# jtdaugherty/flux

Measured on AMD Instinct MI355X. Metric: Msamples/sec on demo2.yml (fixed spp), higher is better.
Workload: dtype f64

## Files before the change

### flux_amd/build.py

```python
import os
import shutil
import subprocess
import sys

ROOT = os.path.dirname(os.path.dirname(os.path.abspath(__file__)))
CSRC = os.path.join(ROOT, "flux_amd", "csrc")
HIP_SOURCES = ["abi.hip", "multi.hip", "tables.hip", "render.hip", "bvh.cpp", "scene_build.cpp", "launch_plan.cpp"]
HIP_HEADERS = ["flux_ctx.h", "scene_build.h", "joining_thread.h", "flux_device.h", "flux_plan.h", "flux_rng.h", "flux_tables.h", "flux_bvh.h", "flux_math.h",
               "flux_math_coeffs.h", "render_body.inc"]
HIP_LIB = os.path.join(ROOT, "flux_amd", "libflux_hip.so")

HIP_FLAGS = ["--offload-arch=gfx950", "-O3", "-std=c++17", "-fPIC", "-shared", "-ffp-contract=off",
             "-fno-fast-math", "-Wall", "-Wno-unused-function",
             "-mllvm", "-disable-machine-licm"]


def _newer(target, deps):
    if not os.path.exists(target):
        return True
    t = os.path.getmtime(target)
    return any(os.path.getmtime(d) > t for d in deps)


def _hipcc():
    for cand in (os.environ.get("HIPCC"), shutil.which("hipcc"), "/opt/rocm/bin/hipcc"):
        if cand and os.path.exists(cand):
            return cand
    raise RuntimeError("hipcc not found (set HIPCC)")


KERNEL_FILES = ["render.hip", "render_body.inc", "tables.hip", "flux_device.h", "flux_plan.h", "flux_bvh.h", "flux_math.h",
                "flux_math_coeffs.h", "flux_rng.h", "flux_tables.h"]


def build_id(extra_flags=()):
    import hashlib

    def digest(names):
        h = hashlib.sha256()
        h.update(" ".join(HIP_FLAGS + list(extra_flags)).encode())
        for n in names:
            path = os.path.join(ROOT, "include", n) if n == "flux_abi.h" else os.path.join(CSRC, n)
            h.update(n.encode() + b"\0")
            with open(path, "rb") as f:
                h.update(f.read())
        return h.hexdigest()[:16]
    return f"lib:{digest(sorted(set(HIP_SOURCES + HIP_HEADERS + ['flux_abi.h'])))} kernels:{digest(KERNEL_FILES)}"


def _id_flag(extra_flags=()):
    return "-DFLUX_BUILD_ID=\"" + build_id(extra_flags) + "\""


def build_variant(out_path, extra_flags, verbose=False):
    srcs = [os.path.join(CSRC, s) for s in HIP_SOURCES]
    flags = [f for f in HIP_FLAGS if not (f == "-ffp-contract=off" and any(x.startswith("-ffp-contract") for x in extra_flags))]
    cmd = [_hipcc()] + flags + list(extra_flags) + [_id_flag(extra_flags), "-o", out_path] + srcs
    if verbose:
        print(" ".join(cmd), file=sys.stderr)
    subprocess.run(cmd, check=True, cwd=CSRC)
    return out_path


def build_hip(force=False, verbose=False):
    srcs = [os.path.join(CSRC, s) for s in HIP_SOURCES]
    deps = srcs + [os.path.join(CSRC, h) for h in HIP_HEADERS] + [os.path.join(ROOT, "include", "flux_abi.h")]
    if not force and not _newer(HIP_LIB, deps):
        return HIP_LIB
    cmd = [_hipcc()] + HIP_FLAGS + [_id_flag(), "-o", HIP_LIB] + srcs
    if verbose:
        print(" ".join(cmd), file=sys.stderr)
    subprocess.run(cmd, check=True, cwd=CSRC)
    return HIP_LIB


HOST_DIR = os.path.join(ROOT, "flux_amd", "host")
HOST_SOURCES = ["flux_host.cpp", "yaml_lite.cpp", "cbor.cpp", "flux_net.cpp"]
HOST_BINARIES = {"flux": "flux_cli.cpp", "flux_host_test": "flux_host_test.cpp", "sampler_debug": "sampler_debug.cpp",
                 "flux_node": "flux_node.cpp"}


def build_host(force=False, verbose=False):
    build_hip(force=False, verbose=verbose)
    outs = []
    common = [os.path.join(HOST_DIR, s) for s in HOST_SOURCES]
# ... 18 lines not shown
```

### flux_amd/csrc/flux_device.h

```cpp
#pragma once
#include <hip/hip_runtime.h>
#include <stdint.h>

#include "flux_bvh.h"


#ifndef FLUX_UNI_SPHERES
#define FLUX_UNI_SPHERES 2
#endif
#ifndef FLUX_BVH_WIDE_MAX_STACK
#define FLUX_BVH_WIDE_MAX_STACK 48
#endif
#ifndef FLUX_MAX_WAVES_PER_PIXEL
#define FLUX_MAX_WAVES_PER_PIXEL 4
#endif
#ifndef FLUX_MIN_SAMPLES_PER_WAVE
#define FLUX_MIN_SAMPLES_PER_WAVE 4096
#endif

namespace flux {

constexpr int kHemiDoubles = 4;
constexpr double kTMin = 0.0005;
constexpr double kPi = 3.14159265358979323846264338327950288;
constexpr double kInvPi = 1.0 / kPi;

constexpr int kShapeSphere = 0;
constexpr int kShapePlane = 1;
constexpr int kShapeDisk = 2;
constexpr int kShapeBox = 3;
constexpr int kMatMatte = 0;
constexpr int kMatEmissive = 1;
constexpr int kMatReflective = 2;
constexpr int kMatGlossy = 3;
constexpr int kMatDielectric = 4;

struct DevShape {
    double px, py, pz;
    double rr;
    double c0x, c0y, c0z;
    double radius;
    double c1x, c1y, c1z;
    double inv;
    int32_t kind;
    int32_t pad0;
    double inv_rad;
    double pad1[2];
};
static_assert(sizeof(DevShape) == 128, "DevShape layout");

struct DevMaterial {
    double fr, fg, fb;
    double exponent;
    double inv_e1;
    int32_t kind;
    int32_t exp_parity;
    double pad1[2];
// ... 77 lines not shown
    const double *hemi;
    const double *gloss;
    const int32_t *rowperm;
    const int32_t *invperm;
    double *out;
    int32_t first_row, row_stride, num_rows;
    int32_t n_mats;
    unsigned long long *stats;
    const DevTri *tris;
    const DevNode *nodes;
    const DevNodeQ *nodesq;
    float bvh_qmin[3], bvh_qstep[3];
    const DevNode4Q *nodes4;
    const DevLeafRec *leaves;
    int32_t bvh4_stack;
    int32_t mat_bits;
    int32_t n_tris;
    int32_t bvh_stack;
    const DevScanSphere *fsph;
    const DevScanPlane *fpln;
    const DevHitRec *frec;
    const DevScanSphere32 *fsph32;
    const DevShape *sshapes;
    int32_t n_sph, n_pln;
    double bvh_mag;
    int32_t set_first, set_stride, set_count, out_by_set;
    int32_t slot_first, slot_stride;
    int32_t glossy_long;
    int32_t self_skip;
    int32_t n_uni, uni_idx[2];
    int32_t unit_dirs;
    int32_t env_short, pad_env;
    double env_radius;
    double t_min, env_deep;
    double env_px, env_py, env_pz, env_rr;
    double env_eps;
    const DevScanSphere32 *f32_half, *f32_top;
    int32_t f32_groups;
    uint32_t f32_valid;
    double fwx, fwy, fwz;
    const double *pxc;
    const DevSetRows *set_rows;
    double exp2c[12];
    const DevScanDisk *fdsk;
    int32_t n_dsk;
    int32_t has_diel;
    const double2 *glossx;
    const int32_t *gx_off;
    int32_t gx_stride, n_gloss_exp;
    const DevScanBox *fbox;
    int32_t n_box;
    int32_t tput_bits;
    const double *tput;
};

__host__ __device__ inline int hit_records(const RenderParams &p) { return p.n_sph + p.n_pln + p.n_dsk + 6 * p.n_box; }

}
```

### flux_amd/csrc/render_body.inc

```

#undef FLUX_STAGE
#if FLUX_FAST
#define FLUX_STAGE() __builtin_amdgcn_sched_barrier(0)
#else
#define FLUX_STAGE() ((void)0)
#endif

struct Ray {
    double ox, oy, oz, dx, dy, dz;
};

typedef const __attribute__((address_space(4))) RenderParams *ParamsInKernarg;
static_assert(sizeof(DevMaterial) % 16 == 0, "the bounce-weight records behind the materials are read as double2");
__device__ __forceinline__ const RenderParams &relaunder_params(uint32_t tick) {
    ParamsInKernarg p = (ParamsInKernarg)__builtin_amdgcn_kernarg_segment_ptr();
    asm("" : "+s"(p) : "s"(tick));
    return *(const RenderParams *)p;
}

__device__ __forceinline__ unsigned long long ballot64(bool b) { return __builtin_amdgcn_ballot_w64(b); }
__device__ __forceinline__ bool any64(bool b) { return __builtin_amdgcn_ballot_w64(b) != 0ull; }
__device__ __forceinline__ bool all64(bool b) { return __builtin_amdgcn_ballot_w64(!b) == 0ull; }

typedef double flux_d2 __attribute__((ext_vector_type(2)));
// ... 348 lines not shown
        filter_pair_step(F, S[0], cand);
    }
    const DevScanSphere32 *g = P.f32_top;
    for (int n = P.f32_groups; n > 0; --n) {
        g -= 4;
        DevScanSphere32 S[4];
#pragma unroll
        for (int j = 0; j < 4; ++j) S[j] = g[j];
#pragma unroll
        for (int j = 3; j >= 0; --j) filter_pair_step(F, S[j], cand);
    }
    return cand;
}

#if FLUX_FAST
__device__ __forceinline__ bool box_z_nan_miss(const RenderParams &P, const Ray &r, int k) {
    const DevShape &S = P.shapes[P.frec[k].orig_id];
    return r.oz == S.c0z || r.oz == S.c1z;
}

__device__ __forceinline__ double sphere_hb(double tx, double ty, double tz, double ux, double uy, double uz) {
    return __builtin_fma(tz, uz, __builtin_fma(ty, uy, tx * ux));
}

__device__ __forceinline__ void scan_disks(const RenderParams &P, const Ray &r, double tmin, int &best, int &best_id, double &tb) {
    for (int j = 0; j < P.n_dsk; ++j) {
        const DevScanDisk &S = P.fdsk[j];
        double t;
        if (disk_hit(S, r, tmin, t) && (best < 0 || t < tb || (t == tb && S.id < best_id))) {
            best = P.n_sph + P.n_pln + j;
            best_id = S.id;
            tb = t;
        }
    }
}

__device__ __forceinline__ void scan_boxes(const RenderParams &P, const Ray &r, double tmin, int &best, int &best_id, double &tb) {
    if (P.n_box <= 0) return;
    const BoxRay A = box_ray(r);
    const int rec0 = P.n_sph + P.n_pln + P.n_dsk;
    for (int j = 0; j < P.n_box; ++j) {
        const DevScanBox &S = P.fbox[j];
        double t;
        int face;
        if (box_shape_hit(S.c0x, S.c0y, S.c0z, S.c1x, S.c1y, S.c1z, r, A, tmin, t, face) &&
            (best < 0 || t < tb || (t == tb && S.id < best_id))) {
            best = rec0 + 6 * j + face;
            best_id = S.id;
            tb = t;
        }
    }
}

template <bool ENV_SHORT = false, bool LDS_SCENE = false, bool MAX32 = false, bool TYP = false, int ZF = -1>
__device__ __forceinline__ void scan_shapes_fast(const RenderParams &P, const Ray &r, int self, int &best, double &tb,
                                                 long long *lap = nullptr, const char *fsph_lds = nullptr) {
    (void)fsph_lds;
    int best_id = -1;
    const double tmin = P.t_min;
    int j0 = 0;
    if (P.n_pln > 0) {
        const DevScanPlane &S = P.fpln[0];
        const double num = (S.px - r.ox) * S.nx + (S.py - r.oy) * S.ny + (S.pz - r.oz) * S.nz;
        const double den = r.dx * S.nx + r.dy * S.ny + r.dz * S.nz;
        const double t = num / den;
        const bool take = t > tmin;
        best = take ? P.n_sph : -1;
        best_id = S.id;
        tb = (ENV_SHORT || take) ? t : tb;
        j0 = 1;
    }
    for (int j = j0; j < P.n_pln; ++j) {
        const DevScanPlane &S = P.fpln[j];
        const double num = (S.px - r.ox) * S.nx + (S.py - r.oy) * S.ny + (S.pz - r.oz) * S.nz;
        const double den = r.dx * S.nx + r.dy * S.ny + r.dz * S.nz;
        const double t = num / den;
        if (t > tmin && (best < 0 || t < tb)) {
            best = P.n_sph + j;
            best_id = S.id;
            tb = t;
        }
    }
    if (!TYP) {
        scan_disks(P, r, tmin, best, best_id, tb);
        scan_boxes(P, r, tmin, best, best_id, tb);
    }
    const bool p_unit_dirs = TYP ? true : P.unit_dirs != 0;
    const bool p_env_short = TYP ? true : P.env_short != 0;
    const int p_n_uni = TYP ? 1 : P.n_uni;
    double rs = 1.0, ux = r.dx, uy = r.dy, uz = r.dz;
    if (!p_unit_dirs) {
        const double dd = r.dx * r.dx + r.dy * r.dy + r.dz * r.dz;
        rs = fastmath::frsqrt(dd);
        ux = r.dx * rs;
        uy = r.dy * rs;
        uz = r.dz * rs;
    }
    const bool zflat = r.dz == 0.0;
    const bool any_zflat = ZF == 0 ? false : any64(zflat);
    const bool f32_filter = (TYP && ENV_SHORT) ? true : P.fsph32 != nullptr;
    float oof;
    const FilterRay32 F32 = filter_ray32_f(r.ox, r.oy, r.oz, ux, uy, uz, oof);
    const bool big = ZF == 0 ? false : !(oof < 1e30f);
    if (ZF != 0 && !(oof < 0.999e6f)) self = -1;
    lap_stamp(lap, 2);
    const int n_groups_end = MAX32 ? ((TYP || P.n_sph > 0) ? 1 : 0) : P.n_sph;
    for (int base = 0; base < n_groups_end; base += 32) {
        const int lim = MAX32 ? P.n_sph : ((P.n_sph - base) < 32 ? (P.n_sph - base) : 32);
        uint32_t cand = 0;
        if (f32_filter) {
            cand = MAX32 ? sphere_filter32_laid_out(P, F32) : sphere_filter32(P, F32, base, lim);
            const uint32_t valid_bits = MAX32 ? P.f32_valid : (lim == 32 ? 0xffffffffu : (1u << lim) - 1u);
            cand = big ? valid_bits : (cand & valid_bits);
            const uint32_t sb = (uint32_t)(self - base);
            cand &= ~(sb < 32u ? 1u << sb : 0u);
        } else
        {
#pragma unroll 4
        for (int k = 0; k < lim; ++k) {
            const DevScanSphere S = P.fsph[base + k];
            const double tx = r.ox - S.px, ty = r.oy - S.py, tz = r.oz - S.pz;
            const double hb = sphere_hb(tx, ty, tz, ux, uy, uz);
            const double c = __builtin_fma(tx, tx, __builtin_fma(ty, ty, __builtin_fma(tz, tz, -S.rr)));
            const double dq = __builtin_fma(hb, hb, -c);
            const int hq = __double2hiint(dq);
            const int hc = __double2hiint(c);
            const int hmin = min(hc, __double2hiint(hb));
            if (hq >= 0 && hmin <= 0) cand |= 1u << k;
        }
        }
        if (any_zflat) {
            if (zflat)
                for (uint32_t m = cand; m;) {
                    const int k = __builtin_ctz(m);
                    m &= m - 1;
                    if (box_z_nan_miss(P, r, base + k)) cand &= ~(1u << k);
                }
        }
        lap_stamp(lap, 3);
        uint32_t todo = cand;
        if (todo) {
            auto record = [&](int k) {
                if constexpr (LDS_SCENE)
                    return *reinterpret_cast<const DevScanSphere *>(fsph_lds + (uint32_t)(base + k) * (uint32_t)sizeof(DevScanSphere));
                else
                    return *reinterpret_cast<const DevScanSphere *>(
                        reinterpret_cast<const char *>(P.fsph) + (uint32_t)(base + k) * (uint32_t)sizeof(DevScanSphere));
            };
            int k = __builtin_ctz(todo);
            todo &= todo - 1;
            DevScanSphere Sk = record(k);
            for (;;) {
                FLUX_TRIP(P, 11);
                FLUX_CENSUS(P, 4);
                const double tx = r.ox - Sk.px, ty = r.oy - Sk.py, tz = r.oz - Sk.pz;
                const double hb = sphere_hb(tx, ty, tz, ux, uy, uz);
                const double c = __builtin_fma(tx, tx, __builtin_fma(ty, ty, __builtin_fma(tz, tz, -Sk.rr)));
                const double dq = __builtin_fma(hb, hb, -c);
                if (dq >= 0.0) {
                    const double e = fastmath::fsqrt_nonneg(dq);
                    double t = (-hb - e) * rs;
                    if (!(t > tmin)) t = (-hb + e) * rs;
                    if (t > tmin) {
                        bool take = best < 0 || t < tb;
                        if (!take && t == tb && best >= P.n_sph) take = P.frec[base + k].orig_id < best_id;
                        if (take) {
                            best = base + k;
                            tb = t;
                        }
                    }
                }
                if (!todo) break;
                k = __builtin_ctz(todo);
                todo &= todo - 1;
                Sk = record(k);
            }
        }
        lap_stamp(lap, 4);
    }
    if (f32_filter) {
        for (int j = 0; j < p_n_uni; ++j) {
            FLUX_CENSUS(P, 5);
            const int k = P.uni_idx[j];
            const DevScanSphere S = TYP ? DevScanSphere{P.env_px, P.env_py, P.env_pz, P.env_rr} : P.fsph[k];
            const double tx = r.ox - S.px, ty = r.oy - S.py, tz = r.oz - S.pz;
            const double hb = sphere_hb(tx, ty, tz, ux, uy, uz);
            const double c = __builtin_fma(tx, tx, __builtin_fma(ty, ty, __builtin_fma(tz, tz, -S.rr)));
            const double dq = __builtin_fma(hb, hb, -c);
            if (ENV_SHORT && p_env_short && p_unit_dirs && !any_zflat) {
                const bool deep = c < P.env_deep;
                const double s = tb + hb;
                const double s2 = s * s;
                const bool close = fabs(dq - s2) <= P.env_eps * (dq + s2);
                if (((ballot64(!deep)) | (ballot64(best >= 0) & ballot64(close))) == 0ull) {
                    if (best < 0 || (s > 0.0 && dq < s2)) {
                        best = k;
                        tb = 2.0 * P.env_radius;
                    }
                    continue;
                }
            }
            const double e = fastmath::fsqrt_nonneg(__builtin_fmax(dq, 0.0));
            double t = (-hb - e) * rs;
            if (!(t > tmin)) t = (-hb + e) * rs;
            bool ok = dq >= 0.0 && t > tmin;
            if (any_zflat) {
                if (zflat && box_z_nan_miss(P, r, k)) ok = false;
            }
            if (ok) {
                bool take = best < 0 || t < tb;
                if (!take && t == tb) take = best >= P.n_sph ? P.frec[k].orig_id < best_id : k < best;
                if (take) {
                    best = k;
                    tb = t;
                }
            }
        }
    }
}
#endif

template <bool STATS, bool TRIS>
__device__ __forceinline__ int scene_hit(const RenderParams &P, const Ray &r, int self, double &t_out, int &slot_out,
                                         int *tstack, int stride, Stats &st) {
    int best = -1;
    int bslot = -1;
    double tb = 0.0;
#if FLUX_FAST
    scan_shapes_fast(P, r, self, best, tb);
    const int best_rec = best;
    if (TRIS) best = best >= 0 ? 0 : -1;
#else
    const double ax = 1.0 / r.dx, ay = 1.0 / r.dy, az = 1.0 / r.dz;
    const double a = r.dx * r.dx + r.dy * r.dy + r.dz * r.dz;
    const double denom = 2.0 * a;
    const auto box_hit_strict = [&](const DevShape &S) {
        double lox = (S.c0x - r.ox) * ax, hix = (S.c1x - r.ox) * ax;
        double loy = (S.c0y - r.oy) * ay, hiy = (S.c1y - r.oy) * ay;
        double loz = (S.c0z - r.oz) * az, hiz = (S.c1z - r.oz) * az;
        double tx_min = ax >= 0.0 ? lox : hix, tx_max = ax >= 0.0 ? hix : lox;
        double ty_min = ay >= 0.0 ? loy : hiy, ty_max = ay >= 0.0 ? hiy : loy;
        double tz_min = az >= 0.0 ? loz : hiz, tz_max = az >= 0.0 ? hiz : loz;
        const double t0 = __builtin_fmax(tx_min, __builtin_fmax(ty_min, tz_min));
        const double t1 = __builtin_fmin(tx_max, __builtin_fmin(ty_max, tz_max));
        return t0 < t1 && t1 > kTMin && !__builtin_isunordered(tz_min, tz_max);
    };
    const auto sphere_hit_strict = [&](const DevShape &S) {
        V3 temp = mk(r.ox - S.px, r.oy - S.py, r.oz - S.pz);
        double b = 2.0 * (temp.x * r.dx + temp.y * r.dy + temp.z * r.dz);
        double c = dot(temp, temp) - S.rr;
        double disc = b * b - 4.0 * a * c;
        if (!(disc < 0.0)) {
            double e = sqrt(disc);
            double t = (-b - e) / denom;
            bool ok = t > kTMin;
            if (!ok) {
                t = (-b + e) / denom;
                ok = t > kTMin;
            }
            if (ok) consider(t, S.pad0, -1, best, bslot, tb);
        }
    };
    if (P.fsph32 != nullptr) {
        for (int j = 0; j < P.n_pln; ++j) {
            const DevScanPlane &S = P.fpln[j];
            double num = (S.px - r.ox) * S.nx + (S.py - r.oy) * S.ny + (S.pz - r.oz) * S.nz;
            double den = r.dx * S.nx + r.dy * S.ny + r.dz * S.nz;
            double t = num / den;
            if (t > kTMin) consider(t, S.id, -1, best, bslot, tb);
        }
        for (int j = 0; j < P.n_dsk; ++j) {
// ... 289 lines not shown
                    if (rdotwi != rdotwi) lobe = rdotwi;
                    const double pdf = lobe * ndotwi;
                    fr *= lobe;
                    fg *= lobe;
                    fb *= lobe;
                    scale = ndotwi / pdf;
                }
            }
        }
    }
    if (p_unit_dirs) {
        const double ss = matte ? 1.0 : __builtin_fma(-0.5, dot(wi, wi), 1.5);
        wi = mk(wi.x * ss, wi.y * ss, wi.z * ss);
    }
    p.self = (p_self_skip && convex && __double2hiint(t) < 0x408f4000 && dot(n, wi) >= 0.0) ? hit : -1;
    if (FIRST) {
        p.tr = fr * scale;
        p.tg = fg * scale;
        p.tb = fb * scale;
    } else {
        p.tr *= fr * scale;
        p.tg *= fg * scale;
        p.tb *= fb * scale;
    }
    p.nb++;
    p.depth++;
    p.r.ox = pt.x;
    p.r.oy = pt.y;
    p.r.oz = pt.z;
    p.r.dx = wi.x;
    p.r.dy = wi.y;
    p.r.dz = wi.z;
}

template <bool LDS_SCENE>
__device__ __forceinline__ int analytic_hit_fields(const RenderParams &P, const Ray &r, int hit, double t, const char *frec_lds, V3 &n,
                                                   int &kind, bool &unit_n, bool &convex, double &fr, double &fg, double &fb,
                                                   double &m_inv_e1, double &ax, double &az) {
    (void)frec_lds;
    const DevHitRec R = *reinterpret_cast<const DevHitRec *>((LDS_SCENE ? frec_lds : reinterpret_cast<const char *>(P.frec)) +
                                                              (uint32_t)hit * (uint32_t)sizeof(DevHitRec));
    kind = R.mat_kind;
    unit_n = R.unit_normal != 0;
    fr = R.fr; fg = R.fg; fb = R.fb; m_inv_e1 = R.inv_e1;
    ax = R.ax; az = R.az;
    const V3 ns = mk(((r.ox - R.cx) + t * r.dx) * R.inv_rad, ((r.oy - R.cy) + t * r.dy) * R.inv_rad,
                     ((r.oz - R.cz) + t * r.dz) * R.inv_rad);
    const bool sph = R.shape_kind == kShapeSphere;
    n = mk(sph ? ns.x : R.cx, sph ? ns.y : R.cy, sph ? ns.z : R.cz);
    convex = sph && R.inv_rad > 0.0;
    return R.orig_id;
}

template <bool STATS, bool TRIS, bool LDS_SCENE = false, bool TYP = false, bool FIRST = false, bool BOUNCE = true>
__device__ __forceinline__ bool shade_hit_fast(const RenderParams &P, Path &p, uint32_t set, uint32_t i, int hit, int slot, double t,
                                               double &Lr, double &Lg, double &Lb, Stats &st, int cz, const char *frec_lds = nullptr) {
    (void)frec_lds;
    (void)cz;
    int bounce = 0;
    const bool is_tri = TRIS && slot >= 0;
    const V3 d = mk(p.r.dx, p.r.dy, p.r.dz);
    const V3 pt = mk(p.r.ox + t * d.x, p.r.oy + t * d.y, p.r.oz + t * d.z);
    V3 n = mk(0.0, 0.0, 1.0);
    int kind = kMatEmissive;
    bool unit_n = true;
    bool convex = false;
    double fr = 0.0, fg = 0.0, fb = 0.0, m_inv_e1 = 0.0, ax = 0.0, az = 0.0;
    if (hit < 0) {
        Lr = P.bgr;
        Lg = P.bgg;
        Lb = P.bgb;
        if (STATS) st.c[6]++;
    } else {
        if (is_tri) {
            const DevTri &T = P.tris[slot];
            const DevMaterial &Mt = P.mats[T.mat];
            p.mat = T.mat;
            n = mk(T.nx, T.ny, T.nz);
            kind = Mt.kind;
            fr = Mt.fr; fg = Mt.fg; fb = Mt.fb; m_inv_e1 = Mt.inv_e1;
            ax = kind == kMatMatte ? 0.0034 : 0.00424;
            az = kind == kMatMatte ? 0.0071 : 0.00764;
        } else {
            p.mat = analytic_hit_fields<LDS_SCENE>(P, p.r, hit, t, frec_lds, n, kind, unit_n, convex, fr, fg, fb, m_inv_e1, ax, az);
        }
        if (kind == kMatEmissive) {
            if (STATS) st.c[5]++;
            const bool front = ((n.x * -1.0) * d.x + (n.y * -1.0) * d.y + (n.z * -1.0) * d.z) > 0.0;
            Lr = fr;
            Lg = fg;
            Lb = fb;
            if (ballot64(!front) != 0ull) {
                Lr = front ? fr : 0.0;
                Lg = front ? fg : 0.0;
                Lb = front ? fb : 0.0;
            }
        } else {
            bounce = 1;
        }
    }
    asm("" : "+v"(bounce));
    if (BOUNCE && bounce) {
        fast_bounce<STATS, TRIS, TYP, FIRST>(P, p, set, i, hit, slot, t, n, d, pt, kind, fr, fg, fb, m_inv_e1, ax, az, unit_n, convex, is_tri, st,
                                            cz);
    }
    return bounce != 0;
}

template <bool STATS, bool TYP>
__device__ __forceinline__ void bounce_parked_hit(const RenderParams &P, Path &p, uint32_t set, uint32_t i, int hit, double t, Stats &st,
                                                  int cz, const char *frec_lds) {
    const V3 d = mk(p.r.dx, p.r.dy, p.r.dz);
    const V3 pt = mk(p.r.ox + t * d.x, p.r.oy + t * d.y, p.r.oz + t * d.z);
    V3 n;
    int kind;
    bool unit_n, convex;
    double fr, fg, fb, m_inv_e1, ax, az;
    p.mat = analytic_hit_fields<true>(P, p.r, hit, t, frec_lds, n, kind, unit_n, convex, fr, fg, fb, m_inv_e1, ax, az);
    fast_bounce<STATS, false, TYP, false>(P, p, set, i, hit, -1, t, n, d, pt, kind, fr, fg, fb, m_inv_e1, ax, az, unit_n, convex, false, st, cz);
}
#endif

template <bool STATS, bool TRIS, bool TWO_PHASE = false, bool LDS_SCENE = false, bool TYP = false>
__device__ __forceinline__ bool shade_hit(const RenderParams &P, Path &p, uint32_t set, uint32_t i, int hit,
                                          int slot, double t, double *stk, int stk_stride, double &Lr,
                                          double &Lg, double &Lb, Stats &st, int cz = 0, const char *frec_lds = nullptr,
                                          const char *mats_lds = nullptr) {
    (void)cz;
    (void)frec_lds;
    (void)mats_lds;
#if FLUX_FAST
    if (TWO_PHASE) return shade_hit_fast<STATS, TRIS>(P, p, set, i, hit, slot, t, Lr, Lg, Lb, st, cz);
#endif
    if (hit < 0) {
        Lr = P.bgr;
        Lg = P.bgg;
        Lb = P.bgb;
        if (STATS) st.c[6]++;
        return false;
    }
    const bool is_tri = TRIS && slot >= 0;
// ... 705 lines not shown
                        const uint32_t *e = hitq_entry(pool, C, nhit - 1u - rank);
                        p.r.ox = lds_dword_pair(e + kHitQOx);
                        p.r.oy = lds_dword_pair(e + kHitQOy);
                        p.r.oz = lds_dword_pair(e + kHitQOz);
                        p.r.dx = lds_dword_pair(e + kHitQDx);
                        p.r.dy = lds_dword_pair(e + kHitQDy);
                        p.r.dz = lds_dword_pair(e + kHitQDz);
                        const double t = lds_dword_pair(e + kHitQT);
                        const int hd = (int)e[kHitQHitDepth];
                        i = e[kHitQSample];
                        const int hit = hd & 0xffff;
                        p.depth = hd >> 16;
                        ml = e[kHitQList];
                        const uint32_t list_bits = __umul24((uint32_t)(p.depth - 1), (uint32_t)hq_bits);
                        if (P.tput != nullptr) {
                            const uint32_t off = __umul24(tput_index(list_bits, ml), (uint32_t)kTputEntryBytes);
                            p.tr = gather_global<double>(P.tput, off);
                            p.tg = gather_global<double>(P.tput, off + 8u);
                            p.tb = gather_global<double>(P.tput, off + 16u);
                        } else {
                            const DevHitRec &R0 = recs[ml & bmask];
                            p.tr = R0.fr;
                            p.tg = R0.fg;
                            p.tb = R0.fb;
#pragma unroll 1
                            for (int k = 1; k < p.depth - 1; ++k) {
                                const DevHitRec &Rk = recs[(ml >> (k * hq_bits)) & bmask];
                                p.tr *= Rk.fr;
                                p.tg *= Rk.fg;
                                p.tb *= Rk.fb;
                            }
                        }
                        ml |= (uint32_t)hit << list_bits;
                        bounce_parked_hit<STATS, TYP>(P, p, set_p, i, hit, t, st, 6, frec_lds);
                    }
                    nhit -= take;
                }
            }
            if (__builtin_expect((nhit | (s_hi - next)) == 0u, 0)) {
                if (!any64(p.depth != kDeadDepth)) break;
            }
            FLUX_TRIP(P, 10);
            const bool live = p.depth != kDeadDepth;
            const bool trace = p.depth <= P.max_depth;
            double Lr = 0.0, Lg = 0.0, Lb = 0.0;
            bool cont = false;
            int hit = -1;
            double t = 0.0;
            if (trace) {
                FLUX_CENSUS(P, 3);
                if (STATS) st.c[1]++;
                const float ofx = (float)p.r.ox, ofy = (float)p.r.oy, ofz = (float)p.r.oz;
                const float oo32 = __builtin_fmaf(ofz, ofz, __builtin_fmaf(ofy, ofy, ofx * ofx));
                if (__builtin_expect((ballot64(p.r.dz == 0.0) | ballot64(!(oo32 < 0.999e6f))) != 0ull, 0))
                    scan_shapes_fast<true, true, MAX32, TYP, 1>(P, p.r, p.self, hit, t, nullptr, fsph_lds);
                else
                    scan_shapes_fast<true, true, MAX32, TYP, 0>(P, p.r, p.self, hit, t, nullptr, fsph_lds);
                cont = shade_hit_fast<STATS, false, true, TYP, false, false>(P, p, set_p, i, hit, -1, t, Lr, Lg, Lb, st, 0, frec_lds);
            }
            if (live && !cont) {
                if (STATS && !trace) st.c[7]++;
                fold_path(p, nullptr, 0, Lr, Lg, Lb);
                sr += Lr;
                sg += Lg;
                sb += Lb;
            }
            const unsigned long long pmask = ballot64(cont);
            if (cont) {
                uint32_t *e = hitq_entry(pool, C, nhit + __builtin_amdgcn_mbcnt_hi((uint32_t)(pmask >> 32),
                                                                                   __builtin_amdgcn_mbcnt_lo((uint32_t)pmask, 0u)));
                lds_dword_pair_store(e + kHitQOx, p.r.ox);
                lds_dword_pair_store(e + kHitQOy, p.r.oy);
                lds_dword_pair_store(e + kHitQOz, p.r.oz);
                lds_dword_pair_store(e + kHitQDx, p.r.dx);
                lds_dword_pair_store(e + kHitQDy, p.r.dy);
                lds_dword_pair_store(e + kHitQDz, p.r.dz);
                lds_dword_pair_store(e + kHitQT, t);
                e[kHitQHitDepth] = (uint32_t)(hit | (p.depth << 16));
                e[kHitQSample] = i;
                e[kHitQList] = ml;
            }
            nhit += (uint32_t)__popcll(pmask);
        }
    }
    if (!HQ && wave_on) {
        unsigned long long cand_mask, in_mask;
        double in_t0;
        pixel_sphere_mask(P, row, col, lane, cand_mask, in_mask, in_t0);

#ifdef FLUX_DEBUG_CLOCK
        long long lap_store[8] = {0, 0, 0, 0, 0, 0, 0, (long long)__builtin_readcyclecounter()};
        long long *lap = lap_store;
#else
        long long *lap = nullptr;
#endif
        uint32_t next = s_lo;
        uint32_t qcount = 0;
        uint32_t i = 0;
        constexpr int kDeadDepth = 0x7fffffff;
        Path p;
        path_begin(p);
        p.depth = kDeadDepth;
        p.sq = make_double2(0.0, 0.0);
        p.r = Ray{0, 0, 0, 0, 0, 1};
        for (;;) {
            const RenderParams &P = relaunder_params(next + qcount);
            uint32_t set_p = set;
            unsigned long long cand_p = cand_mask, in_p = in_mask;
            asm("" : "+s"(set_p) : "s"(next));
            asm("" : "+s"(cand_p), "+s"(in_p) : "s"(next));
            auto pop = [&]() {
// ... 877 lines not shown
```

### flux_amd/csrc/scene_build.cpp

```cpp
#include "scene_build.h"

#include <algorithm>
#include <cmath>
#include <cstdio>
#include <cstdlib>
#include <cstring>

#include "joining_thread.h"

namespace flux {

namespace {

void normalize3(const double in[3], double out[3]) {
    double len = std::sqrt(in[0] * in[0] + in[1] * in[1] + in[2] * in[2]);
    out[0] = in[0] / len;
    out[1] = in[1] / len;
    out[2] = in[2] / len;
}
void cross3(const double a[3], const double b[3], double o[3]) {
    o[0] = a[1] * b[2] - a[2] * b[1];
    o[1] = a[2] * b[0] - a[0] * b[2];
    o[2] = a[0] * b[1] - a[1] * b[0];
}
// ... 170 lines not shown
    const double half_w = (double)W * 0.5, half_h = (double)H * 0.5;
    for (uint32_t x = 0; x < W; x++) pxc[x] = (double)(int32_t)x - half_w;
    for (uint32_t y = 0; y < H; y++) pxc[W + y] = (double)((int32_t)H - (int32_t)y) - half_h;

    rp.n_sph = (int32_t)fsph.size();
    rp.n_pln = (int32_t)fpln.size();
    rp.n_dsk = (int32_t)fdsk.size();
    rp.n_box = (int32_t)fbox.size();
    std::vector<const DevHitRec *> frec_all;
    for (const auto *v : {&frec_s, &frec_p, &frec_d, &frec_b})
        for (const DevHitRec &hr : *v) frec_all.push_back(&hr);
    auto same_bits = [](double a, double b) { return std::memcmp(&a, &b, sizeof(double)) == 0; };
    auto slot_of = [&](double v) {
        size_t k = 0;
        while (k < h.gx_inv_e1.size() && !same_bits(h.gx_inv_e1[k], v)) k++;
        return k;
    };
    {
        std::vector<const DevHitRec *> yaml(frec_all);
        std::sort(yaml.begin(), yaml.end(), [](const DevHitRec *a, const DevHitRec *b) { return a->orig_id < b->orig_id; });
        for (const DevHitRec *hr : yaml)
            if (hr->mat_kind == kMatGlossy && h.gx_inv_e1.size() <= (size_t)kGlossExpSlots && slot_of(hr->inv_e1) == h.gx_inv_e1.size())
                h.gx_inv_e1.push_back(hr->inv_e1);
    }
    rp.n_gloss_exp = (int32_t)h.gx_inv_e1.size();
    h.gx_off.assign(frec_all.size() + 1, 0);
    for (const DevHitRec &hr : frec_p)
        if (!hr.unit_normal) rp.glossy_long = 1;
    for (const DevHitRec &hr : frec_d)
        if (!hr.unit_normal) rp.glossy_long = 1;
    rp.unit_dirs = rp.glossy_long ? 0 : 1;
    rp.self_skip = rp.glossy_long ? 0 : 1;
    if (rp.n_gloss_exp >= 1 && rp.n_gloss_exp <= kGlossExpSlots && !rp.glossy_long) {
        rp.gx_stride = 16 * rp.n_gloss_exp;
        for (size_t k = 0; k < frec_all.size(); k++)
            if (frec_all[k]->mat_kind == kMatGlossy) h.gx_off[k] = 16 * (int32_t)slot_of(frec_all[k]->inv_e1);
    }
    for (const DevScanSphere &sp : fsph)
        if (!(std::fabs(sp.px) < 1e3 && std::fabs(sp.py) < 1e3 && std::fabs(sp.pz) < 1e3 && sp.rr < 1e6)) rp.self_skip = 0;
    const int inverted = (int)std::count_if(frec_s.begin(), frec_s.end(), [](const DevHitRec &hr) { return hr.inv_rad < 0.0; });
    if (rp.n_uni == 1 && inverted == 1 && frec_s[rp.uni_idx[0]].mat_kind == kMatEmissive) {
        const double rad = std::sqrt(fsph[rp.uni_idx[0]].rr);
        if (rad > 1e-3 && rad < 1e6) {
            rp.env_short = 1;
            rp.env_radius = rad * (1.0 + 1e-12);
        }
    }
    rp.t_min = kTMin;
    rp.env_deep = -(4.0 * kTMin) * rp.env_radius;
    rp.env_eps = 1e-9;
    if (rp.n_uni == 1) {
        const DevScanSphere &es = fsph[rp.uni_idx[0]];
        rp.env_px = es.px; rp.env_py = es.py; rp.env_pz = es.pz; rp.env_rr = es.rr;
    }
    rp.f32_valid = fsph.size() >= 32 ? 0xffffffffu : (1u << fsph.size()) - 1u;
    if (h.filter32 && fsph.size() <= 32) {
        int pairs = ((int)fsph.size() + 1) >> 1;
        const int rem = pairs & 3;
        if (rem == 1 || rem == 2) {
            h.f32_half = pairs - rem;
            pairs -= rem;
        } else if (rem == 3) {
            pairs += 1;
        }
        rp.f32_groups = pairs / 4;
        h.f32_top = pairs;
    }
}

}

void build_tput_table(const HostScene &h, int bits, int max_depth, std::vector<double> &out) {
    const DevHitRec *rec = reinterpret_cast<const DevHitRec *>(h.fscene.data() + h.fs.rec);
    const uint32_t n_rec = (uint32_t)hit_records(h.rp);
    out.assign(((size_t)2 << (bits * (max_depth - 1))) * 3, 0.0);
    for (uint32_t e = 0; e < n_rec; e++) {
        double *t = &out[(size_t)tput_index((uint32_t)bits, e) * 3];
        t[0] = rec[e].fr; t[1] = rec[e].fg; t[2] = rec[e].fb;
    }
    std::vector<uint32_t> heads(n_rec), lists;
    for (uint32_t e = 0; e < n_rec; e++) heads[e] = e;
    for (int n = 2; n < max_depth; n++) {
        const uint32_t head_bits = (uint32_t)(bits * (n - 1));
        lists.clear();
        lists.reserve(heads.size() * n_rec);
        for (uint32_t e = 0; e < n_rec; e++)
            for (const uint32_t head : heads) {
                const uint32_t ml = head | (e << head_bits);
                const double *a = &out[(size_t)tput_index(head_bits, head) * 3];
                double *t = &out[(size_t)tput_index(head_bits + (uint32_t)bits, ml) * 3];
                t[0] = a[0] * rec[e].fr; t[1] = a[1] * rec[e].fg; t[2] = a[2] * rec[e].fb;
                lists.push_back(ml);
            }
        heads.swap(lists);
    }
}

namespace {
int build_meshes(const flux_scene_desc &scene, HostScene &h, std::string &error) {
    const size_t ns = (size_t)scene.num_shapes;
    std::vector<size_t> first((size_t)scene.num_meshes + 1, 0);
    for (size_t m = 0; m < (size_t)scene.num_meshes; m++) first[m + 1] = first[m] + (size_t)scene.meshes[m].num_triangles;
    if ((uint64_t)first.back() * sizeof(DevTri) >= (1ull << 32)) {
        char buf[160];
        std::snprintf(buf, sizeof(buf), "%zu triangles exceed the %llu a context can hold", first.back(),
                      (unsigned long long)((1ull << 32) / sizeof(DevTri)));
// ... 151 lines not shown
```

Baseline: 52030.

## Add f32 env-sphere verdict and carry hit facing into emissive shading

Adds a conservative single-precision test, with an error margin, that decides whether the enclosing emissive environment sphere wins or loses against the current best hit. When it is conclusive for the whole wavefront, the f64 quadratic is skipped. The sphere scan also records a facing sign taken from the discriminant's high word, so emissive shading can decide front/back from that sign instead of an f64 normal dot product. This aims to cut f64 ALU work on the bounce path, but adds f32 work, extra branches and register pressure, and the margins have to be strictly conservative for results to stay correct.

```diff
diff --git a/flux_amd/build.py b/flux_amd/build.py
--- a/flux_amd/build.py
+++ b/flux_amd/build.py
@@ -7,7 +7,7 @@
 CSRC = os.path.join(ROOT, "flux_amd", "csrc")
 HIP_SOURCES = ["abi.hip", "multi.hip", "tables.hip", "render.hip", "bvh.cpp", "scene_build.cpp", "launch_plan.cpp"]
 HIP_HEADERS = ["flux_ctx.h", "scene_build.h", "joining_thread.h", "flux_device.h", "flux_plan.h", "flux_rng.h", "flux_tables.h", "flux_bvh.h", "flux_math.h",
-               "flux_math_coeffs.h", "render_body.inc"]
+               "flux_math_coeffs.h", "flux_env_verdict.h", "render_body.inc"]
 HIP_LIB = os.path.join(ROOT, "flux_amd", "libflux_hip.so")
 
 HIP_FLAGS = ["--offload-arch=gfx950", "-O3", "-std=c++17", "-fPIC", "-shared", "-ffp-contract=off",
@@ -30,7 +30,7 @@
 
 
 KERNEL_FILES = ["render.hip", "render_body.inc", "tables.hip", "flux_device.h", "flux_plan.h", "flux_bvh.h", "flux_math.h",
-                "flux_math_coeffs.h", "flux_rng.h", "flux_tables.h"]
+                "flux_math_coeffs.h", "flux_rng.h", "flux_tables.h", "flux_env_verdict.h"]
 
 
 def build_id(extra_flags=()):
diff --git a/flux_amd/csrc/flux_device.h b/flux_amd/csrc/flux_device.h
--- a/flux_amd/csrc/flux_device.h
+++ b/flux_amd/csrc/flux_device.h
@@ -3,6 +3,7 @@
 #include <stdint.h>
 
 #include "flux_bvh.h"
+#include "flux_env_verdict.h"
 
 
 #ifndef FLUX_UNI_SPHERES
@@ -186,6 +187,7 @@
     int32_t n_box;
     int32_t tput_bits;
     const double *tput;
+    EnvSphere32 env32;
 };
 
 __host__ __device__ inline int hit_records(const RenderParams &p) { return p.n_sph + p.n_pln + p.n_dsk + 6 * p.n_box; }
diff --git a/flux_amd/csrc/flux_env_verdict.h b/flux_amd/csrc/flux_env_verdict.h
--- /dev/null
+++ b/flux_amd/csrc/flux_env_verdict.h
@@ -0,0 +1,57 @@
+#pragma once
+#include <cmath>
+
+#if defined(__HIPCC__) || defined(__CUDACC__)
+#define FLUX_ENV_HD __host__ __device__ inline
+#else
+#define FLUX_ENV_HD inline
+#endif
+
+namespace flux {
+
+constexpr int kEnvUndecided = 0, kEnvWins = 1, kEnvLoses = 2;
+constexpr float kEnvMargin32 = 8e-6f;
+
+struct EnvSphere32 {
+    float npx, npy, npz;
+    float ppr;
+    float mag;
+    float deep;
+};
+
+inline EnvSphere32 env_sphere32(double px, double py, double pz, double rr, double deep) {
+    const double pp = px * px + py * py + pz * pz;
+    float d = (float)deep;
+    if ((double)d > deep) d = std::nextafterf(d, -INFINITY);
+    return EnvSphere32{-(float)px, -(float)py, -(float)pz, (float)(pp - rr), (float)(pp + rr), d};
+}
+
+struct EnvRay32 {
+    float hb2;
+    float cm;
+    float cp;
+};
+
+FLUX_ENV_HD EnvRay32 env_ray32(const EnvSphere32 &E, float o2x, float o2y, float o2z, float ux, float uy, float uz, float ou, float oo) {
+    const float hb = __builtin_fmaf(E.npx, ux, __builtin_fmaf(E.npy, uy, __builtin_fmaf(E.npz, uz, ou)));
+    const float c = __builtin_fmaf(E.npx, o2x, __builtin_fmaf(E.npy, o2y, __builtin_fmaf(E.npz, o2z, oo))) + E.ppr;
+    const float m = kEnvMargin32 * (oo + E.mag);
+    return EnvRay32{2.0f * hb, c - m, c + m};
+}
+
+FLUX_ENV_HD void env_g32(const EnvRay32 &R, float tb, float &g_lo, float &g_hi) {
+    g_lo = __builtin_fmaf(tb, __builtin_fmaf(1.0f - kEnvMargin32, tb, R.hb2), R.cm);
+    g_hi = __builtin_fmaf(tb, __builtin_fmaf(1.0f + kEnvMargin32, tb, R.hb2), R.cp);
+}
+
+FLUX_ENV_HD int env_verdict32(const EnvSphere32 &E, const EnvRay32 &R, float tb, bool has_best) {
+    if (!(R.cp < E.deep)) return kEnvUndecided;
+    if (!has_best) return kEnvWins;
+    float g_lo, g_hi;
+    env_g32(R, tb, g_lo, g_hi);
+    if (g_lo > 0.0f) return kEnvWins;
+    if (g_hi < 0.0f) return kEnvLoses;
+    return kEnvUndecided;
+}
+
+}
diff --git a/flux_amd/csrc/render_body.inc b/flux_amd/csrc/render_body.inc
--- a/flux_amd/csrc/render_body.inc
+++ b/flux_amd/csrc/render_body.inc
@@ -424,10 +424,22 @@
     }
 }
 
-template <bool ENV_SHORT = false, bool LDS_SCENE = false, bool MAX32 = false, bool TYP = false, int ZF = -1>
+constexpr int kFaceDqHi = 0x3d719799;
+constexpr float kFaceEnvFront = 1.8446744073709552e19f;
+__device__ __forceinline__ float sphere_facing(double dq, bool near_root) {
+    const float hq = __int_as_float(__double2hiint(dq));
+    return near_root ? -hq : hq;
+}
+__device__ __forceinline__ bool facing_known(int facing) { return (facing & 0x7fffffff) > kFaceDqHi; }
+__device__ __forceinline__ bool facing_front(int facing, int inv_rad_hi) { return (facing ^ inv_rad_hi) < 0; }
+
+template <bool ENV_SHORT = false, bool LDS_SCENE = false, bool MAX32 = false, bool TYP = false, int ZF = -1, bool FACING = false>
 __device__ __forceinline__ void scan_shapes_fast(const RenderParams &P, const Ray &r, int self, int &best, double &tb,
-                                                 long long *lap = nullptr, const char *fsph_lds = nullptr) {
+                                                 long long *lap = nullptr, const char *fsph_lds = nullptr, int *facing = nullptr) {
     (void)fsph_lds;
+    (void)facing;
+    constexpr bool FACE = FACING && ZF == 0;
+    float face = 0.0f;
     int best_id = -1;
     const double tmin = P.t_min;
     int j0 = 0;
@@ -474,6 +486,10 @@
     float oof;
     const FilterRay32 F32 = filter_ray32_f(r.ox, r.oy, r.oz, ux, uy, uz, oof);
     const bool big = ZF == 0 ? false : !(oof < 1e30f);
+    constexpr bool ENV32 = ENV_SHORT && ZF == 0;
+    EnvRay32 E32 = EnvRay32{0.0f, 0.0f, 0.0f};
+    if (ENV32 && p_env_short && p_unit_dirs)
+        E32 = env_ray32(P.env32, F32.o2x2[0], F32.o2y2[0], F32.o2z2[0], F32.u_x[0], F32.u_y[0], F32.u_z[0], F32.ou2[0], oof);
     if (ZF != 0 && !(oof < 0.999e6f)) self = -1;
     lap_stamp(lap, 2);
     const int n_groups_end = MAX32 ? ((TYP || P.n_sph > 0) ? 1 : 0) : P.n_sph;
@@ -532,6 +548,7 @@
                 if (dq >= 0.0) {
                     const double e = fastmath::fsqrt_nonneg(dq);
                     double t = (-hb - e) * rs;
+                    const float face_k = sphere_facing(dq, t > tmin);
                     if (!(t > tmin)) t = (-hb + e) * rs;
                     if (t > tmin) {
                         bool take = best < 0 || t < tb;
@@ -539,6 +556,7 @@
                         if (take) {
                             best = base + k;
                             tb = t;
+                            if (FACE) face = face_k;
                         }
                     }
                 }
@@ -554,6 +572,18 @@
         for (int j = 0; j < p_n_uni; ++j) {
             FLUX_CENSUS(P, 5);
             const int k = P.uni_idx[j];
+            if (ENV32 && p_env_short && p_unit_dirs) {
+                float g_lo, g_hi;
+                env_g32(E32, (float)tb, g_lo, g_hi);
+                if ((ballot64(!(E32.cp < P.env32.deep)) | (ballot64(best >= 0) & ballot64(!(g_lo > 0.0f)) & ballot64(!(g_hi < 0.0f)))) == 0ull) {
+                    if (best < 0 || g_lo > 0.0f) {
+                        best = k;
+                        tb = 2.0 * P.env_radius;
+                        if (FACE) face = kFaceEnvFront;
+                    }
+                    continue;
+                }
+            }
             const DevScanSphere S = TYP ? DevScanSphere{P.env_px, P.env_py, P.env_pz, P.env_rr} : P.fsph[k];
             const double tx = r.ox - S.px, ty = r.oy - S.py, tz = r.oz - S.pz;
             const double hb = sphere_hb(tx, ty, tz, ux, uy, uz);
@@ -568,6 +598,7 @@
                     if (best < 0 || (s > 0.0 && dq < s2)) {
                         best = k;
                         tb = 2.0 * P.env_radius;
+                        if (FACE) face = kFaceEnvFront;
                     }
                     continue;
                 }
@@ -585,10 +616,12 @@
                 if (take) {
                     best = k;
                     tb = t;
-                }
-            }
-        }
-    }
+                    if (FACE) face = 0.0f;
+                }
+            }
+        }
+    }
+    if (FACING) *facing = (FACE && (TYP || P.self_skip != 0)) ? __float_as_int(face) : 0;
 }
 #endif
 
@@ -984,10 +1017,12 @@
     return R.orig_id;
 }
 
-template <bool STATS, bool TRIS, bool LDS_SCENE = false, bool TYP = false, bool FIRST = false, bool BOUNCE = true>
+template <bool STATS, bool TRIS, bool LDS_SCENE = false, bool TYP = false, bool FIRST = false, bool BOUNCE = true, bool FACING = false>
 __device__ __forceinline__ bool shade_hit_fast(const RenderParams &P, Path &p, uint32_t set, uint32_t i, int hit, int slot, double t,
-                                               double &Lr, double &Lg, double &Lb, Stats &st, int cz, const char *frec_lds = nullptr) {
+                                               double &Lr, double &Lg, double &Lb, Stats &st, int cz, const char *frec_lds = nullptr,
+                                               int facing = 0) {
     (void)frec_lds;
+    (void)facing;
     (void)cz;
     int bounce = 0;
     const bool is_tri = TRIS && slot >= 0;
@@ -1018,7 +1053,13 @@
         }
         if (kind == kMatEmissive) {
             if (STATS) st.c[5]++;
-            const bool front = ((n.x * -1.0) * d.x + (n.y * -1.0) * d.y + (n.z * -1.0) * d.z) > 0.0;
+            bool front;
+            if (FACING && ballot64(!facing_known(facing)) == 0ull) {
+                const DevHitRec &R = *reinterpret_cast<const DevHitRec *>(frec_lds + (uint32_t)hit * (uint32_t)sizeof(DevHitRec));
+                front = facing_front(facing, reinterpret_cast<const int *>(&R.inv_rad)[1]);
+            } else {
+                front = ((n.x * -1.0) * d.x + (n.y * -1.0) * d.y + (n.z * -1.0) * d.z) > 0.0;
+            }
             Lr = fr;
             Lg = fg;
             Lb = fb;
@@ -1830,11 +1871,12 @@
                 if (STATS) st.c[1]++;
                 const float ofx = (float)p.r.ox, ofy = (float)p.r.oy, ofz = (float)p.r.oz;
                 const float oo32 = __builtin_fmaf(ofz, ofz, __builtin_fmaf(ofy, ofy, ofx * ofx));
+                int facing;
                 if (__builtin_expect((ballot64(p.r.dz == 0.0) | ballot64(!(oo32 < 0.999e6f))) != 0ull, 0))
-                    scan_shapes_fast<true, true, MAX32, TYP, 1>(P, p.r, p.self, hit, t, nullptr, fsph_lds);
+                    scan_shapes_fast<true, true, MAX32, TYP, 1, true>(P, p.r, p.self, hit, t, nullptr, fsph_lds, &facing);
                 else
-                    scan_shapes_fast<true, true, MAX32, TYP, 0>(P, p.r, p.self, hit, t, nullptr, fsph_lds);
-                cont = shade_hit_fast<STATS, false, true, TYP, false, false>(P, p, set_p, i, hit, -1, t, Lr, Lg, Lb, st, 0, frec_lds);
+                    scan_shapes_fast<true, true, MAX32, TYP, 0, true>(P, p.r, p.self, hit, t, nullptr, fsph_lds, &facing);
+                cont = shade_hit_fast<STATS, false, true, TYP, false, false, true>(P, p, set_p, i, hit, -1, t, Lr, Lg, Lb, st, 0, frec_lds, facing);
             }
             if (live && !cont) {
                 if (STATS && !trace) st.c[7]++;
diff --git a/flux_amd/csrc/scene_build.cpp b/flux_amd/csrc/scene_build.cpp
--- a/flux_amd/csrc/scene_build.cpp
+++ b/flux_amd/csrc/scene_build.cpp
@@ -246,6 +246,7 @@
     if (rp.n_uni == 1) {
         const DevScanSphere &es = fsph[rp.uni_idx[0]];
         rp.env_px = es.px; rp.env_py = es.py; rp.env_pz = es.pz; rp.env_rr = es.rr;
+        rp.env32 = env_sphere32(es.px, es.py, es.pz, es.rr, rp.env_deep);
     }
     rp.f32_valid = fsph.size() >= 32 ? 0xffffffffu : (1u << fsph.size()) - 1u;
     if (h.filter32 && fsph.size() <= 32) {
diff --git a/profiles/r11_scan_verdicts/env_block_after.s b/profiles/r11_scan_verdicts/env_block_after.s
--- /dev/null
+++ b/profiles/r11_scan_verdicts/env_block_after.s
@@ -0,0 +1,81 @@
+.LBB24_193:
+	s_or_b64 exec, exec, s[8:9]
+	v_fma_f32 v1, s22, v46, v52
+	v_fmac_f32_e32 v1, s21, v44
+	v_fmac_f32_e32 v2, s22, v10
+	v_fmac_f32_e32 v1, s20, v6
+	v_fmac_f32_e32 v2, s21, v4
+	v_add_f32_e32 v3, s23, v1
+	v_add_f32_e32 v1, s74, v52
+	v_mul_f32_e32 v4, 0x370637bd, v1
+	v_fmac_f32_e32 v2, s20, v0
+	s_load_dword s2, s[68:69], 0x31c
+	s_load_dword s14, s[68:69], 0x1d4
+	v_sub_f32_e32 v1, v3, v4
+	v_add_f32_e32 v0, v2, v2
+	v_add_f32_e32 v2, v3, v4
+	v_cvt_f32_f64_e32 v3, v[8:9]
+	v_fmamk_f32 v4, v3, 0x3f7fff7a, v0
+	v_fmac_f32_e32 v1, v3, v4
+	v_fmamk_f32 v0, v3, 0x3f800043, v0
+	s_waitcnt lgkmcnt(0)
+	v_cmp_ngt_f32_e32 vcc, s2, v2
+	v_fmac_f32_e32 v2, v3, v0
+	v_cmp_lt_i32_e64 s[2:3], -1, v54
+	v_cmp_nlt_f32_e64 s[4:5], 0, v1
+	s_and_b64 s[4:5], s[4:5], s[2:3]
+	v_cmp_ngt_f32_e64 s[2:3], 0, v2
+	s_and_b64 s[2:3], s[4:5], s[2:3]
+	s_or_b64 s[2:3], s[2:3], vcc
+	s_cmp_lg_u64 s[2:3], 0
+	s_cselect_b64 s[4:5], -1, 0
+	s_and_b64 vcc, exec, s[4:5]
+	s_cbranch_vccz .LBB24_195
+	s_andn2_b64 vcc, exec, s[4:5]
+	s_cbranch_vccz .LBB24_198
+	s_branch .LBB24_216
+.LBB24_195:
+	v_cmp_gt_i32_e32 vcc, 0, v54
+	v_cmp_lt_f32_e64 s[2:3], 0, v1
+	s_or_b64 s[8:9], vcc, s[2:3]
+	s_and_saveexec_b64 s[2:3], s[8:9]
+	s_cbranch_execz .LBB24_197
+	s_load_dwordx2 s[8:9], s[68:69], 0x1e8
+	v_mov_b32_e32 v47, 0x5f800000
+	v_mov_b32_e32 v54, s14
+	s_waitcnt lgkmcnt(0)
+	v_add_f64 v[8:9], s[8:9], s[8:9]
+.LBB24_197:
+	s_or_b64 exec, exec, s[2:3]
+	s_andn2_b64 vcc, exec, s[4:5]
+	s_cbranch_vccnz .LBB24_216
+.LBB24_198:
+	s_load_dwordx8 s[16:23], s[68:69], 0x1f8
+	s_load_dwordx4 s[8:11], s[68:69], 0x218
+	v_cmp_lt_i32_e64 s[2:3], -1, v54
+	s_waitcnt lgkmcnt(0)
+	v_add_f64 v[2:3], v[18:19], -s[18:19]
+	v_add_f64 v[6:7], v[24:25], -s[22:23]
+	v_add_f64 v[4:5], v[20:21], -s[20:21]
+	v_mul_f64 v[0:1], v[12:13], v[2:3]
+	v_fma_f64 v[10:11], v[6:7], v[6:7], -s[8:9]
+	v_fmac_f64_e32 v[0:1], v[4:5], v[14:15]
+	v_fmac_f64_e32 v[10:11], v[4:5], v[4:5]
+	v_fmac_f64_e32 v[0:1], v[6:7], v[16:17]
+	v_fmac_f64_e32 v[10:11], v[2:3], v[2:3]
+	v_fma_f64 v[2:3], v[0:1], v[0:1], -v[10:11]
+	v_add_f64 v[4:5], v[8:9], v[0:1]
+	v_fma_f64 v[44:45], v[4:5], v[4:5], v[2:3]
+	v_fma_f64 v[6:7], -v[4:5], v[4:5], v[2:3]
+	v_mul_f64 v[44:45], s[10:11], v[44:45]
+	v_cmp_le_f64_e64 s[4:5], |v[6:7]|, v[44:45]
+	v_cmp_ngt_f64_e32 vcc, s[16:17], v[10:11]
+	s_and_b64 s[4:5], s[4:5], s[2:3]
+	s_or_b64 s[4:5], s[4:5], vcc
+	s_cmp_lg_u64 s[4:5], 0
+	s_cselect_b64 s[4:5], -1, 0
+	s_and_b64 vcc, exec, s[4:5]
+	s_cbranch_vccz .LBB24_200
+	s_andn2_b64 vcc, exec, s[4:5]
+	s_cbranch_vccz .LBB24_205
+	s_branch .LBB24_216
diff --git a/profiles/r11_scan_verdicts/env_block_before.s b/profiles/r11_scan_verdicts/env_block_before.s
--- /dev/null
+++ b/profiles/r11_scan_verdicts/env_block_before.s
@@ -0,0 +1,27 @@
+.LBB24_191:
+	s_or_b64 exec, exec, s[6:7]
+	s_load_dwordx8 s[16:23], s[68:69], 0x1f8
+	s_load_dword s14, s[68:69], 0x1d4
+	s_load_dwordx4 s[8:11], s[68:69], 0x218
+	v_cmp_lt_i32_e64 s[2:3], -1, v54
+	s_waitcnt lgkmcnt(0)
+	v_add_f64 v[2:3], v[18:19], -s[18:19]
+	v_add_f64 v[6:7], v[20:21], -s[20:21]
+	v_mul_f64 v[4:5], v[12:13], v[2:3]
+	v_add_f64 v[8:9], v[24:25], -s[22:23]
+	v_fmac_f64_e32 v[4:5], v[6:7], v[14:15]
+	v_fmac_f64_e32 v[4:5], v[8:9], v[16:17]
+	v_fma_f64 v[8:9], v[8:9], v[8:9], -s[8:9]
+	v_fmac_f64_e32 v[8:9], v[6:7], v[6:7]
+	v_fmac_f64_e32 v[8:9], v[2:3], v[2:3]
+	v_fma_f64 v[2:3], v[4:5], v[4:5], -v[8:9]
+	v_add_f64 v[6:7], v[0:1], v[4:5]
+	v_fma_f64 v[44:45], v[6:7], v[6:7], v[2:3]
+	v_fma_f64 v[10:11], -v[6:7], v[6:7], v[2:3]
+	v_mul_f64 v[44:45], s[10:11], v[44:45]
+	v_cmp_le_f64_e64 s[6:7], |v[10:11]|, v[44:45]
+	v_cmp_ngt_f64_e32 vcc, s[16:17], v[8:9]
+	s_and_b64 s[2:3], s[6:7], s[2:3]
+	s_or_b64 s[2:3], s[2:3], vcc
+	s_cmp_lg_u64 s[2:3], 0
+	s_cbranch_scc0 .LBB24_201
diff --git a/profiles/r11_scan_verdicts/facing_block_after.s b/profiles/r11_scan_verdicts/facing_block_after.s
--- /dev/null
+++ b/profiles/r11_scan_verdicts/facing_block_after.s
@@ -0,0 +1,68 @@
+	s_movk_i32 s4, 0x60
+	v_mul_lo_u32 v0, v54, s4
+	v_add_u32_e32 v46, 0x60, v0
+	ds_read_b64 v[44:45], v46 offset:64
+	v_mov_b32_e32 v4, 1
+	v_mov_b64_e32 v[10:11], 0
+	v_mov_b64_e32 v[2:3], 0
+	v_mov_b64_e32 v[0:1], 0
+	s_waitcnt lgkmcnt(0)
+	v_cmp_eq_u32_e32 vcc, 1, v45
+	s_and_saveexec_b64 s[4:5], vcc
+	s_cbranch_execz .LBB24_224
+	ds_read2_b64 v[4:7], v46 offset0:2 offset1:3
+	ds_read2_b64 v[0:3], v46 offset0:4 offset1:5
+	ds_read_b64 v[10:11], v46 offset:48
+	v_and_b32_e32 v45, 0x7ffffffe, v47
+	s_mov_b32 s6, 0x3d71979a
+	v_cmp_gt_u32_e32 vcc, s6, v45
+	s_cbranch_vccz .LBB24_231
+	ds_read2_b64 v[48:51], v46 offset1:1
+	s_waitcnt lgkmcnt(3)
+	v_add_f64 v[52:53], v[24:25], -v[4:5]
+	v_fmac_f64_e32 v[52:53], v[16:17], v[8:9]
+	v_cmp_eq_u32_e32 vcc, 0, v44
+	v_mul_f64 v[52:53], v[6:7], v[52:53]
+	s_waitcnt lgkmcnt(0)
+	v_add_f64 v[56:57], v[18:19], -v[48:49]
+	v_add_f64 v[60:61], v[20:21], -v[50:51]
+	v_fmac_f64_e32 v[56:57], v[12:13], v[8:9]
+	v_fmac_f64_e32 v[60:61], v[14:15], v[8:9]
+	v_mul_f64 v[56:57], v[56:57], v[6:7]
+	v_mul_f64 v[60:61], v[6:7], v[60:61]
+	v_cndmask_b32_e32 v45, v49, v57, vcc
+	v_cndmask_b32_e32 v44, v48, v56, vcc
+	v_cndmask_b32_e32 v49, v51, v61, vcc
+	v_cndmask_b32_e32 v48, v50, v60, vcc
+	v_cndmask_b32_e32 v5, v5, v53, vcc
+	v_cndmask_b32_e32 v4, v4, v52, vcc
+	v_mul_f64 v[44:45], v[12:13], v[44:45]
+	v_fma_f64 v[44:45], v[14:15], -v[48:49], -v[44:45]
+	v_mul_f64 v[4:5], v[16:17], v[4:5]
+	v_cmp_gt_f64_e64 s[6:7], v[44:45], v[4:5]
+	s_cbranch_execnz .LBB24_221
+.LBB24_220:
+	s_waitcnt lgkmcnt(2)
+	v_xor_b32_e32 v4, v47, v7
+	v_cmp_gt_i32_e32 vcc, 0, v4
+	s_andn2_b64 s[6:7], s[6:7], exec
+	s_and_b64 s[8:9], vcc, exec
+	s_or_b64 s[6:7], s[6:7], s[8:9]
+.LBB24_221:
+	s_xor_b64 s[8:9], s[6:7], -1
+	s_waitcnt lgkmcnt(2)
+	v_cndmask_b32_e64 v4, 0, 1, s[8:9]
+	v_cmp_ne_u32_e32 vcc, 0, v4
+	s_cbranch_vccz .LBB24_223
+	s_waitcnt lgkmcnt(0)
+	v_cndmask_b32_e64 v11, 0, v11, s[6:7]
+	v_cndmask_b32_e64 v10, 0, v10, s[6:7]
+	v_cndmask_b32_e64 v3, 0, v3, s[6:7]
+	v_cndmask_b32_e64 v2, 0, v2, s[6:7]
+	v_cndmask_b32_e64 v1, 0, v1, s[6:7]
+	v_cndmask_b32_e64 v0, 0, v0, s[6:7]
+.LBB24_223:
+	v_mov_b32_e32 v4, 0
+.LBB24_224:
+	s_or_b64 exec, exec, s[4:5]
+.LBB24_225:
diff --git a/profiles/r11_scan_verdicts/facing_block_before.s b/profiles/r11_scan_verdicts/facing_block_before.s
--- /dev/null
+++ b/profiles/r11_scan_verdicts/facing_block_before.s
@@ -0,0 +1,54 @@
+	s_movk_i32 s4, 0x60
+	v_mul_lo_u32 v0, v10, s4
+	v_add_u32_e32 v9, 0x60, v0
+	ds_read_b32 v0, v9 offset:68
+	v_mov_b32_e32 v8, 1
+	v_mov_b64_e32 v[6:7], 0
+	v_mov_b64_e32 v[2:3], 0
+	s_waitcnt lgkmcnt(0)
+	v_cmp_eq_u32_e32 vcc, 1, v0
+	v_mov_b64_e32 v[0:1], 0
+	s_and_saveexec_b64 s[4:5], vcc
+	s_cbranch_execz .LBB24_212
+	ds_read2_b64 v[44:47], v9 offset0:2 offset1:3
+	ds_read2_b64 v[0:3], v9 offset0:4 offset1:5
+	ds_read_b64 v[6:7], v9 offset:48
+	ds_read_b32 v11, v9 offset:64
+	ds_read2_b64 v[48:51], v9 offset1:1
+	s_waitcnt lgkmcnt(4)
+	v_add_f64 v[8:9], v[24:25], -v[44:45]
+	v_fmac_f64_e32 v[8:9], v[16:17], v[4:5]
+	v_mul_f64 v[8:9], v[46:47], v[8:9]
+	s_waitcnt lgkmcnt(1)
+	v_cmp_eq_u32_e32 vcc, 0, v11
+	s_nop 1
+	v_cndmask_b32_e32 v9, v45, v9, vcc
+	v_cndmask_b32_e32 v8, v44, v8, vcc
+	s_waitcnt lgkmcnt(0)
+	v_add_f64 v[44:45], v[20:21], -v[50:51]
+	v_fmac_f64_e32 v[44:45], v[14:15], v[4:5]
+	v_mul_f64 v[44:45], v[46:47], v[44:45]
+	v_cndmask_b32_e32 v45, v51, v45, vcc
+	v_cndmask_b32_e32 v44, v50, v44, vcc
+	v_add_f64 v[50:51], v[18:19], -v[48:49]
+	v_fmac_f64_e32 v[50:51], v[12:13], v[4:5]
+	v_mul_f64 v[46:47], v[46:47], v[50:51]
+	v_cndmask_b32_e32 v47, v49, v47, vcc
+	v_cndmask_b32_e32 v46, v48, v46, vcc
+	v_mul_f64 v[46:47], v[12:13], v[46:47]
+	v_fma_f64 v[44:45], v[14:15], -v[44:45], -v[46:47]
+	v_mul_f64 v[8:9], v[16:17], v[8:9]
+	v_cmp_ngt_f64_e32 vcc, v[44:45], v[8:9]
+	s_cbranch_vccz .LBB24_211
+	s_nop 0
+	v_cndmask_b32_e64 v7, v7, 0, vcc
+	v_cndmask_b32_e64 v6, v6, 0, vcc
+	v_cndmask_b32_e64 v3, v3, 0, vcc
+	v_cndmask_b32_e64 v2, v2, 0, vcc
+	v_cndmask_b32_e64 v1, v1, 0, vcc
+	v_cndmask_b32_e64 v0, v0, 0, vcc
+.LBB24_211:
+	v_mov_b32_e32 v8, 0
+.LBB24_212:
+	s_or_b64 exec, exec, s[4:5]
+.LBB24_213:
```

After: 53790, median of 6. 1.03x the previous value.
